# JiehongLin/SAM-6D

Measured on NVIDIA H100. Metric: poses/sec, higher is better.
Workload: dtype bf16

## Files before the change

### sam6d_b200/csrc/attn_tc.cu

```cuda
#include "epilogue.cuh"
#include "tc.cuh"

namespace {

constexpr int QT = 128, MAXK = 256;
constexpr int CONSUMERS = 256, NUM_THREADS = CONSUMERS + 128;
constexpr int REL_SLAB = 32 * 128;
constexpr int SCR_LD = 64;

struct AttnArgs {
  const float* bias;
  const void* rel_blob;
  const float* rel_unused;
  const void* q_rows;
  long long q_ld;
  int q_col0;
  const float* bv;
  void* out;
  long long out_ld;
  int H, Sq, Sk, N1;
  int Hs, Ws;
  int k_col0;
  float scale;
  int k_brows, k_row0, v_col0;
  float* lse;
  long long bias_ld;
};

template <int D>
__host__ __device__ constexpr int qkp_bytes(int N1) {
  return ((((D + 63) / 64) * (QT + N1) * 128 > 4 * QT * 128 ? ((D + 63) / 64) * (QT + N1) * 128 : 4 * QT * 128) + 1023) & ~1023;
}

template <int D, int BIAS_MODE, typename OT>
__global__ void __launch_bounds__(NUM_THREADS, 1) attn_tc_kernel(const __grid_constant__ CUtensorMap tmQ, const __grid_constant__ CUtensorMap tmK,
                                                const __grid_constant__ CUtensorMap tmVt, AttnArgs a) {
  constexpr int DS = (D + 63) / 64;
  constexpr int Q_SLAB = QT * 128, V_SLAB = D * 128, P_SLAB = QT * 128;
  const int K_SLAB = a.N1 * 128;
  extern __shared__ __align__(1024) uint8_t smem_raw[];
  uint8_t* smem = reinterpret_cast<uint8_t*>((reinterpret_cast<uintptr_t>(smem_raw) + 1023) & ~(uintptr_t)1023);
  uint8_t* q_s = smem;
  uint8_t* k_s = q_s + DS * Q_SLAB;
  uint8_t* p_s = smem;
  uint8_t* v_s = smem + qkp_bytes<D>(a.N1);
  uint8_t* rel_s = v_s + 4 * V_SLAB;
  float* scr = reinterpret_cast<float*>(rel_s + 2 * DS * REL_SLAB);
  __shared__ __align__(8) uint64_t load_bar;

  const int tid = threadIdx.x, warp = tid >> 5, lane = tid & 31;
  const int n0 = blockIdx.x * QT, h = blockIdx.y, b = blockIdx.z;
  const int nslab = (a.N1 + 63) / 64;

  if (tid == 0) {
    tc::mbar_init(&load_bar, 1);
    tc::mbar_fence_init();
  }
  s6_pdl_trigger();
  __syncthreads();
  s6_pdl_wait();

  if (warp >= CONSUMERS / 32) {
    tc::producer_regs();
    if (tid == CONSUMERS) {
      uint32_t bytes = (uint32_t)(DS * (QT * 128) + DS * (a.N1 * 128) + nslab * V_SLAB);
      if (BIAS_MODE == 2) bytes += 2 * DS * REL_SLAB;
      tc::mbar_arrive_expect_tx(&load_bar, bytes);
      if (BIAS_MODE == 2) tc::bulk_load_1d(rel_s, a.rel_blob, 2 * DS * REL_SLAB, &load_bar);
#pragma unroll
      for (int s = 0; s < DS; ++s) {
        tc::tma_load_2d(&tmQ, &load_bar, q_s + s * Q_SLAB, a.q_col0 + h * D + s * 64, b * a.Sq + n0);
        tc::tma_load_2d(&tmK, &load_bar, k_s + s * K_SLAB, a.k_col0 + h * D + s * 64, b * a.k_brows + a.k_row0);
      }
      for (int s = 0; s < nslab; ++s) tc::tma_load_2d(&tmVt, &load_bar, v_s + s * V_SLAB, a.v_col0 + s * 64, (b * a.H + h) * D);
    }
    return;
  }
  tc::consumer_regs();
  const int wg = warp >> 2, w = warp & 3;
  const int Sk = a.Sk;
  tc::mbar_wait(&load_bar, 0);
  float sacc[MAXK / 2];
  {
    const uint32_t q_addr = tc::smem_u32(q_s) + wg * (64 * 128), k_addr = tc::smem_u32(k_s);
    tc::wg_fence();
#pragma unroll
    for (int k = 0; k < D / 16; ++k) {
      const int sl = k >> 2, kk = k & 3;
      tc::wgmma_bf16<MAXK>(sacc, tc::wg_desc(q_addr + sl * Q_SLAB + kk * 32), tc::wg_desc(k_addr + sl * K_SLAB + kk * 32), k ? 1u : 0u);
    }
    tc::wg_commit();
    if (BIAS_MODE == 2) {
      float tacc[2][16];
#pragma unroll
      for (int t = 0; t < 2; ++t)
#pragma unroll
        for (int k = 0; k < D / 16; ++k) {
          const int sl = k >> 2, kk = k & 3;
          tc::wgmma_bf16<32>(tacc[t], tc::wg_desc(q_addr + sl * Q_SLAB + kk * 32),
                             tc::wg_desc(tc::smem_u32(rel_s + (t * DS + sl) * REL_SLAB) + kk * 32), k ? 1u : 0u);
        }
      tc::wg_commit();
      tc::wg_wait<0>();
#pragma unroll
      for (int t = 0; t < 2; ++t)
#pragma unroll
        for (int e = 0; e < 16; ++e) scr[(wg * 64 + tc::frag_row(e, w, lane)) * SCR_LD + t * 32 + tc::frag_col(e, lane)] = tacc[t][e];
      tc::named_bar(1 + wg, 128);
    } else {
      tc::wg_wait<0>();
    }
  }
  float mx[2] = {-INFINITY, -INFINITY};
#pragma unroll
  for (int hr = 0; hr < 2; ++hr) {
    const int r = wg * 64 + tc::frag_row(2 * hr, w, lane), n = n0 + r, nq = min(n, a.Sq - 1);
    const float* brow = nullptr;
    if (BIAS_MODE == 1) brow = a.bias + (((size_t)b * a.H + h) * a.Sq + nq) * Sk;
    if (BIAS_MODE == 4) brow = a.bias + (((size_t)b * a.H + h) * a.Sq + nq) * a.bias_ld;
    const float* trow = (BIAS_MODE == 2) ? scr + r * SCR_LD : nullptr;
    const int qh = (BIAS_MODE == 2) ? nq / a.Ws : 0, qw = (BIAS_MODE == 2) ? nq % a.Ws : 0;
#pragma unroll
    for (int j = 0; j < MAXK / 8; ++j) {
      const int col = tc::frag_col(4 * j, lane);
      float bb[2] = {0.f, 0.f};
      if (BIAS_MODE == 4 && col < Sk) { const float2 t = __ldg(reinterpret_cast<const float2*>(brow + col)); bb[0] = t.x; bb[1] = t.y; }
#pragma unroll
      for (int e = 0; e < 2; ++e) {
        const int c = col + e;
        float x = -INFINITY;
        if (c < Sk) {
          x = sacc[4 * j + 2 * hr + e];
          if (BIAS_MODE == 1) x += __ldg(brow + c);
          if (BIAS_MODE == 4) x += bb[e];
          x *= a.scale;
          if (BIAS_MODE == 2) { const int kh = c / a.Ws, kw = c - kh * a.Ws; x += trow[qh - kh + a.Hs - 1] + trow[32 + qw - kw + a.Ws - 1]; }
          mx[hr] = fmaxf(mx[hr], x);
        }
        sacc[4 * j + 2 * hr + e] = x;
      }
    }
    mx[hr] = tc::quad_max(mx[hr]);
  }
  tc::named_bar(3, CONSUMERS);
  float sum[2] = {0.f, 0.f};
#pragma unroll
  for (int j = 0; j < MAXK / 8; ++j) {
#pragma unroll
    for (int hr = 0; hr < 2; ++hr) {
      const int r = wg * 64 + tc::frag_row(2 * hr, w, lane), col = tc::frag_col(4 * j, lane);
      const float p0 = (col < Sk) ? __expf(sacc[4 * j + 2 * hr] - mx[hr]) : 0.f;
      const float p1 = (col + 1 < Sk) ? __expf(sacc[4 * j + 2 * hr + 1] - mx[hr]) : 0.f;
      sum[hr] += p0 + p1;
      *reinterpret_cast<uint32_t*>(p_s + (col >> 6) * P_SLAB + tc::sw128_offset(r, col & 63)) = tc::pack_bf16(p0, p1);
    }
  }
  tc::fence_proxy_async_smem();
  tc::named_bar(1 + wg, 128);
  float oacc[D / 2];
  {
    const uint32_t p_addr = tc::smem_u32(p_s) + wg * (64 * 128), v_addr = tc::smem_u32(v_s);
    tc::wg_fence();
    const int ksteps = a.N1 / 16;
    for (int k = 0; k < ksteps; ++k) {
      const int sl = k >> 2, kk = k & 3;
      tc::wgmma_bf16<D>(oacc, tc::wg_desc(p_addr + sl * P_SLAB + kk * 32), tc::wg_desc(v_addr + sl * V_SLAB + kk * 32), k ? 1u : 0u);
    }
    tc::wg_commit();
    tc::wg_wait<0>();
  }
  const int m_lim = b * a.Sq + a.Sq;
#pragma unroll
  for (int hr = 0; hr < 2; ++hr) {
    const float t = tc::quad_sum(sum[hr]), inv = 1.f / t;
    const int n = n0 + wg * 64 + tc::frag_row(2 * hr, w, lane), row = b * a.Sq + n;
    if (a.lse && n < a.Sq && (lane & 3) == 0) a.lse[((size_t)b * a.H + h) * a.Sq + n] = mx[hr] + __logf(t);
    if (row >= m_lim) continue;
    OT* orow = reinterpret_cast<OT*>(a.out) + (size_t)row * a.out_ld + h * D;
#pragma unroll
    for (int j = 0; j < D / 8; ++j) {
      const int col = tc::frag_col(4 * j, lane);
      float o0 = oacc[4 * j + 2 * hr] * inv, o1 = oacc[4 * j + 2 * hr + 1] * inv;
      if (a.bv) { o0 += __ldg(a.bv + h * D + col); o1 += __ldg(a.bv + h * D + col + 1); }
      epi::st2(orow + col, o0, o1);
    }
  }
}

template <int D, int BM, typename OT>
int launch(const CUtensorMap& tq, const CUtensorMap& tk, const CUtensorMap& tv, const AttnArgs& a, int B, cudaStream_t st) {
  constexpr int DS = (D + 63) / 64;
  size_t smem = (size_t)qkp_bytes<D>(a.N1) + (size_t)4 * D * 128 + 1024;
  if (BM == 2) smem += (size_t)2 * DS * REL_SLAB + (size_t)QT * SCR_LD * sizeof(float);
  if (smem > 227 * 1024) return S6_EINVAL;
  auto kern = attn_tc_kernel<D, BM, OT>;
  cudaError_t e = cudaFuncSetAttribute(kern, cudaFuncAttributeMaxDynamicSharedMemorySize, (int)smem);
  if (e != cudaSuccess) return (int)e;
  dim3 grid(s6_cdiv(a.Sq, QT), a.H, B);
  cudaError_t le = s6_launch_pdl(kern, grid, dim3(NUM_THREADS), smem, st, tq, tk, tv, a);
  if (le != cudaSuccess) return (int)le;
  return (int)cudaGetLastError();
}

__global__ void __launch_bounds__(256) transpose_tokens_kernel(const __nv_bfloat16* __restrict__ src, long long ld, int col0, int C,
                                                               int L, int N1, __nv_bfloat16* __restrict__ out) {
  __shared__ __nv_bfloat16 tile[64][66];
  const int w = blockIdx.z, c0 = blockIdx.y * 64, l0 = blockIdx.x * 64;
  const int tx = threadIdx.x & 63, ty = threadIdx.x >> 6;
  s6_pdl_trigger();
  s6_pdl_wait();
  for (int i = ty; i < 64; i += 4) {
    const int l = l0 + i, c = c0 + tx;
    tile[i][tx] = (l < L && c < C) ? src[((size_t)w * L + l) * ld + col0 + c] : __float2bfloat16(0.f);
  }
  __syncthreads();
  for (int i = ty; i < 64; i += 4) {
    const int c = c0 + i, l = l0 + tx;
    if (c < C && l < N1) out[((size_t)w * C + c) * N1 + l] = tile[tx][i];
  }
}

}

S6_API int sam6d_transpose_tokens_bf16(const void* src, long long ld, int col0, int C, int nB, int L, int N1, void* out, void* stream) {
  S6_REQUIRE(src && out && nB >= 0 && C > 0 && L > 0 && N1 >= L);
  if (nB == 0) return 0;
  S6_REQUIRE(nB <= 65535);
  dim3 grid(s6_cdiv(N1, 64), s6_cdiv(C, 64), nB);
  S6_CHECK(s6_launch_pdl(transpose_tokens_kernel, grid, dim3(256), 0, s6_stream(stream), reinterpret_cast<const __nv_bfloat16*>(src), ld,
                         col0, C, L, N1, reinterpret_cast<__nv_bfloat16*>(out)));
  S6_LAUNCH_CHECK();
  return 0;
}

namespace {
}

namespace {
int attn_tc_launch(const void* Q, long long q_ld, int q_col0, const void* K, long long k_ld, int k_col0, const void* Vt,
                   long long vt_ld, int B, int H, int Sq, int Sk, int head_dim, int bias_mode, const float* bias,
                   const void* rel_h, const float* rel_w, int Hs, int Ws, const float* bv, float scale, void* out,
                   int out_is_bf16, long long out_ld, int k_brows, int k_row0, int v_col0, float* lse, void* stream,
                   long long bias_ld = 0) {
  S6_REQUIRE(Q && K && Vt && out && B >= 0 && H > 0 && Sq > 0 && Sk > 0 && Sk <= MAXK);
  S6_REQUIRE((head_dim == 64 || head_dim == 80) && bias_mode >= 0 && bias_mode <= 4 && bias_mode != 3);
  if (bias_mode == 4)
    S6_REQUIRE(bias && head_dim == 64 && bias_ld >= Sk && (bias_ld % 4) == 0 && (reinterpret_cast<uintptr_t>(bias) & 15) == 0);
  S6_REQUIRE((q_ld % 8) == 0 && (k_ld % 8) == 0 && (vt_ld % 8) == 0 && (q_col0 % 8) == 0 && (k_col0 % 8) == 0);
  S6_REQUIRE(k_brows >= k_row0 + Sk && k_row0 >= 0 && v_col0 >= 0 && (v_col0 % 8) == 0);
  if (bias_mode == 1) S6_REQUIRE(bias != nullptr);
  if (bias_mode == 2) S6_REQUIRE(rel_h && Hs > 0 && Ws > 0 && Hs <= 16 && Ws <= 16 && Hs * Ws == Sk && Sq == Sk && (reinterpret_cast<uintptr_t>(rel_h) & 15) == 0);
  if (B == 0) return 0;
  S6_REQUIRE(B <= 65535 && H <= 65535);
  const int N1 = (Sk + 15) & ~15;
  S6_REQUIRE(vt_ld >= v_col0 + N1);
  CUtensorMap tq, tk, tv;
  int rc = tc::make_map_2d(&tq, Q, (long long)B * Sq, q_ld, q_ld, 64, QT);
  if (rc) return rc;
  rc = tc::make_map_2d(&tk, K, (long long)B * k_brows, k_ld, k_ld, 64, N1);
  if (rc) return rc;
  rc = tc::make_map_2d(&tv, Vt, (long long)B * H * head_dim, vt_ld, vt_ld, 64, head_dim);
  if (rc) return rc;
  AttnArgs a{bias, rel_h, rel_w, Q, q_ld, q_col0, bv, out, out_ld, H, Sq, Sk, N1, Hs, Ws, k_col0, scale, k_brows, k_row0, v_col0, lse, bias_ld};
  cudaStream_t st = s6_stream(stream);
#define ATT_LAUNCH(DD, MM) (out_is_bf16 ? launch<DD, MM, __nv_bfloat16>(tq, tk, tv, a, B, st) : launch<DD, MM, float>(tq, tk, tv, a, B, st))
  if (head_dim == 64) {
    if (bias_mode == 0) return ATT_LAUNCH(64, 0);
    if (bias_mode == 1) return ATT_LAUNCH(64, 1);
    if (bias_mode == 4) return ATT_LAUNCH(64, 4);
    return ATT_LAUNCH(64, 2);
  }
  if (bias_mode == 0) return ATT_LAUNCH(80, 0);
  if (bias_mode == 1) return ATT_LAUNCH(80, 1);
  return ATT_LAUNCH(80, 2);
#undef ATT_LAUNCH
}

__global__ void __launch_bounds__(256) attn_merge_key_kernel(const __nv_bfloat16* __restrict__ Q, long long q_ld, int q_col0,
                                                             const __nv_bfloat16* __restrict__ K, long long k_ld, int k_col0, int k_brows,
                                                             int key_row, const __nv_bfloat16* __restrict__ Vt, long long vt_ld, int key_col,
                                                             const float* __restrict__ lse, int B, int H, int Sq, float scale,
                                                             __nv_bfloat16* __restrict__ out, long long out_ld) {
  const long long w = (long long)blockIdx.x * 8 + (threadIdx.x >> 5);
  const int lane = threadIdx.x & 31;
  s6_pdl_trigger();
  s6_pdl_wait();
  if (w >= (long long)B * Sq * H) return;
  const int h = (int)(w % H);
  const long long bn = w / H;
  const int n = (int)(bn % Sq), b = (int)(bn / Sq);
  const __nv_bfloat162 q2 = *reinterpret_cast<const __nv_bfloat162*>(Q + (size_t)bn * q_ld + q_col0 + h * 64 + lane * 2);
  const __nv_bfloat162 k2 = *reinterpret_cast<const __nv_bfloat162*>(K + ((size_t)b * k_brows + key_row) * k_ld + k_col0 + h * 64 + lane * 2);
  float s = __bfloat162float(q2.x) * __bfloat162float(k2.x) + __bfloat162float(q2.y) * __bfloat162float(k2.y);
  s = warp_sum(s) * scale;
  const float l = lse[((size_t)b * H + h) * Sq + n];
  const float m = fmaxf(l, s), wp = __expf(l - m), wc = __expf(s - m), inv = 1.f / (wp + wc);
  const __nv_bfloat16* vrow = Vt + ((size_t)(b * H + h) * 64 + lane * 2) * vt_ld + key_col;
  const float v0 = __bfloat162float(vrow[0]), v1 = __bfloat162float(vrow[vt_ld]);
  __nv_bfloat162* o = reinterpret_cast<__nv_bfloat162*>(out + (size_t)bn * out_ld + h * 64 + lane * 2);
  const __nv_bfloat162 o2 = *o;
  *o = __floats2bfloat162_rn((wp * __bfloat162float(o2.x) + wc * v0) * inv, (wp * __bfloat162float(o2.y) + wc * v1) * inv);
}
}

S6_API int sam6d_attn_tc(const void* Q, long long q_ld, int q_col0, const void* K, long long k_ld, int k_col0, const void* Vt,
                         long long vt_ld, int B, int H, int Sq, int Sk, int head_dim, int bias_mode, const float* bias,
                         const void* rel_h, const float* rel_w, int Hs, int Ws, const float* bv, float scale, void* out,
                         int out_is_bf16, long long out_ld, void* stream) {
  return attn_tc_launch(Q, q_ld, q_col0, K, k_ld, k_col0, Vt, vt_ld, B, H, Sq, Sk, head_dim, bias_mode, bias, rel_h, rel_w, Hs, Ws, bv,
                        scale, out, out_is_bf16, out_ld, Sk, 0, 0, nullptr, stream);
}

S6_API int sam6d_attn_tc_bias_ld(const void* Q, long long q_ld, int q_col0, const void* K, long long k_ld, int k_col0, const void* Vt,
                                 long long vt_ld, int B, int H, int Sq, int Sk, int head_dim, const float* bias, long long bias_ld,
                                 float scale, void* out, int out_is_bf16, long long out_ld, void* stream) {
  return attn_tc_launch(Q, q_ld, q_col0, K, k_ld, k_col0, Vt, vt_ld, B, H, Sq, Sk, head_dim, 4, bias, nullptr, nullptr, 0, 0, nullptr,
                        scale, out, out_is_bf16, out_ld, Sk, 0, 0, nullptr, stream, bias_ld);
}

S6_API int sam6d_attn_tc_ex(const void* Q, long long q_ld, int q_col0, const void* K, long long k_ld, int k_col0, const void* Vt,
                            long long vt_ld, int B, int H, int Sq, int Sk, int head_dim, float scale, int k_brows, int k_row0, int v_col0,
                            float* lse, void* out, int out_is_bf16, long long out_ld, void* stream) {
  return attn_tc_launch(Q, q_ld, q_col0, K, k_ld, k_col0, Vt, vt_ld, B, H, Sq, Sk, head_dim, 0, nullptr, nullptr, nullptr, 0, 0, nullptr,
                        scale, out, out_is_bf16, out_ld, k_brows, k_row0, v_col0, lse, stream);
}

S6_API int sam6d_attn_merge_key(const void* Q, long long q_ld, int q_col0, const void* K, long long k_ld, int k_col0, int k_brows,
                                int key_row, const void* Vt, long long vt_ld, int key_col, const float* lse, int B, int H, int Sq,
                                float scale, void* out, long long out_ld, void* stream) {
  S6_REQUIRE(Q && K && Vt && lse && out && B >= 0 && H > 0 && Sq > 0 && (q_ld % 2) == 0 && (k_ld % 2) == 0 && (out_ld % 2) == 0 &&
             (q_col0 % 2) == 0 && (k_col0 % 2) == 0);
  if (B == 0) return 0;
  const long long warps = (long long)B * Sq * H;
  S6_CHECK(s6_launch_pdl(attn_merge_key_kernel, dim3(s6_cdiv(warps, 8)), dim3(256), 0, s6_stream(stream),
                         reinterpret_cast<const __nv_bfloat16*>(Q), q_ld, q_col0, reinterpret_cast<const __nv_bfloat16*>(K), k_ld, k_col0,
                         k_brows, key_row, reinterpret_cast<const __nv_bfloat16*>(Vt), vt_ld, key_col, lse, B, H, Sq, scale,
                         reinterpret_cast<__nv_bfloat16*>(out), out_ld));
  S6_LAUNCH_CHECK();
  return 0;
}
```

### sam6d_b200/csrc/geo_lut.cu

```cuda
#include <cuda_bf16.h>

#include "common.cuh"

namespace {

__device__ __forceinline__ uint32_t bf2_pack(float lo, float hi) {
  __nv_bfloat162 h = __floats2bfloat162_rn(lo, hi);
  return *reinterpret_cast<uint32_t*>(&h);
}

__device__ __forceinline__ void lut_pos(float x, float inv_h, int nent, int& row, float& t) {
  const float u = x * inv_h;
  int i = (int)u;
  i = max(0, min(i, nent - 2));
  t = u - (float)i;
  row = i * 32;
}
__device__ __forceinline__ void lut_lerp_f32(const uint4* __restrict__ tab, int row, float t, float v[8]) {
  const uint4 lo = tab[row], hi = tab[row + 32];
  const uint32_t l[4] = {lo.x, lo.y, lo.z, lo.w}, h[4] = {hi.x, hi.y, hi.z, hi.w};
#pragma unroll
  for (int k = 0; k < 4; ++k) {
    const float l0 = __uint_as_float(l[k] << 16), l1 = __uint_as_float(l[k] & 0xffff0000u);
    const float h0 = __uint_as_float(h[k] << 16), h1 = __uint_as_float(h[k] & 0xffff0000u);
    v[2 * k] = fmaf(t, h0 - l0, l0);
    v[2 * k + 1] = fmaf(t, h1 - l1, l1);
  }
}
__device__ __forceinline__ void unpack8(const uint4& a, float v[8]) {
  const uint32_t w[4] = {a.x, a.y, a.z, a.w};
#pragma unroll
  for (int k = 0; k < 4; ++k) { v[2 * k] = __uint_as_float(w[k] << 16); v[2 * k + 1] = __uint_as_float(w[k] & 0xffff0000u); }
}

__device__ __noinline__ uint4 slow_distance(float x, const float* __restrict__ div_term, const uint4* __restrict__ WdT,
                                            const float* __restrict__ bias, int lane) {
  float e[8];
#pragma unroll
  for (int q = 0; q < 4; ++q) sincosf(x * div_term[lane * 4 + q], &e[2 * q], &e[2 * q + 1]);
  float acc[8];
#pragma unroll
  for (int c = 0; c < 8; ++c) acc[c] = bias[lane * 8 + c];
  for (int s = 0; s < 32; ++s) {
#pragma unroll
    for (int q = 0; q < 8; ++q) {
      const float v = __shfl_sync(0xffffffffu, e[q], s);
      const uint4 w = WdT[(size_t)(s * 8 + q) * 32 + lane];
      const uint32_t ww[4] = {w.x, w.y, w.z, w.w};
#pragma unroll
      for (int i = 0; i < 4; ++i) {
        acc[2 * i] = fmaf(v, __uint_as_float(ww[i] << 16), acc[2 * i]);
        acc[2 * i + 1] = fmaf(v, __uint_as_float(ww[i] & 0xffff0000u), acc[2 * i + 1]);
      }
    }
  }
  return make_uint4(bf2_pack(acc[0], acc[1]), bf2_pack(acc[2], acc[3]), bf2_pack(acc[4], acc[5]), bf2_pack(acc[6], acc[7]));
}

constexpr int LUT_THREADS = 512, UNROLL = 2;
__global__ void __launch_bounds__(LUT_THREADS, 1) geo_embed_lut_kernel(const float4* __restrict__ T, long long npairs, int S,
                                                                      const uint4* __restrict__ tabA_g, int na, float inv_ha,
                                                                      const uint4* __restrict__ tabD_g, int nd, float inv_hd,
                                                                      const uint4* __restrict__ far, const float* __restrict__ div_term,
                                                                      const uint4* __restrict__ WdT, const float* __restrict__ bias,
                                                                      uint4* __restrict__ E) {
  extern __shared__ __align__(16) uint8_t smem_raw[];
  uint4* tabA = reinterpret_cast<uint4*>(smem_raw);
  uint4* tabD = tabA + na * 32;
  const int tid = threadIdx.x, lane = tid & 31, warp = tid >> 5;
  for (int u = tid; u < na * 32; u += LUT_THREADS) tabA[u] = tabA_g[u];
  for (int u = tid; u < nd * 32; u += LUT_THREADS) tabD[u] = tabD_g[u];
  __syncthreads();
  const float d_limit = (float)(nd - 1) / inv_hd;
  const long long nblocks = (npairs + 31) / 32;
  const long long SS = (long long)S * S;
  for (long long blk = (long long)blockIdx.x * (LUT_THREADS / 32) + warp; blk < nblocks; blk += (long long)gridDim.x * (LUT_THREADS / 32)) {
    const long long base = blk * 32;
    const int cnt = (int)min(32LL, npairs - base);
    float4 tv = make_float4(0.f, 0.f, 0.f, 0.f);
    if (lane < cnt) tv = T[base + lane];
    int r0, r1, r2, r3;
    float t0, t1, t2, t3;
    lut_pos(tv.x, inv_ha, na, r0, t0);
    lut_pos(tv.y, inv_ha, na, r1, t1);
    lut_pos(tv.z, inv_ha, na, r2, t2);
    lut_pos(tv.w, inv_hd, nd, r3, t3);
    if (!(tv.w < d_limit)) r3 = -1;
    const uint4* tabA_l = tabA + lane;
    const uint4* tabD_l = tabD + lane;
#pragma unroll UNROLL
    for (int j = 0; j < cnt; ++j) {
      const int q0 = __shfl_sync(0xffffffffu, r0, j), q1 = __shfl_sync(0xffffffffu, r1, j);
      const int q2 = __shfl_sync(0xffffffffu, r2, j), q3 = __shfl_sync(0xffffffffu, r3, j);
      const float w0 = __shfl_sync(0xffffffffu, t0, j), w1 = __shfl_sync(0xffffffffu, t1, j);
      const float w2 = __shfl_sync(0xffffffffu, t2, j), w3 = __shfl_sync(0xffffffffu, t3, j);
      uint4 dv;
      const bool in_table = q3 >= 0;
      if (!in_table) {
        const long long p = base + j;
        const long long c = p / SS;
        const int rem = (int)(p - c * SS), n = rem / S, m = rem - n * S;
        if (n == 0) dv = far[((c * 2 + 0) * S + m) * 32 + lane];
        else if (m == 0) dv = far[((c * 2 + 1) * S + n) * 32 + lane];
        else dv = slow_distance(__shfl_sync(0xffffffffu, tv.w, j), div_term, WdT, bias, lane);
      }
      float f0[8], f1[8], f2[8], fd[8];
      lut_lerp_f32(tabA_l, q0, w0, f0);
      lut_lerp_f32(tabA_l, q1, w1, f1);
      lut_lerp_f32(tabA_l, q2, w2, f2);
      if (in_table) lut_lerp_f32(tabD_l, q3, w3, fd);
      else unpack8(dv, fd);
#pragma unroll
      for (int k = 0; k < 8; ++k) fd[k] += fmaxf(fmaxf(f0[k], f1[k]), f2[k]);
      const uint4 o = make_uint4(bf2_pack(fd[0], fd[1]), bf2_pack(fd[2], fd[3]), bf2_pack(fd[4], fd[5]), bf2_pack(fd[6], fd[7]));
      E[(base + j) * 32 + lane] = o;
    }
  }
}

}

S6_API int sam6d_geo_embed_lut(const float* T, long long clouds, int S, const void* tabA, int na, float inv_ha, const void* tabD, int nd,
                               float inv_hd, const void* far, const float* div_term, const void* WdT_bf16, const float* bias, void* E,
                               void* stream) {
  S6_REQUIRE(T && tabA && tabD && far && div_term && WdT_bf16 && bias && E && clouds >= 0 && S > 0 && na >= 2 && nd >= 2);
  S6_REQUIRE(inv_ha > 0.f && inv_hd > 0.f && (long long)(na + nd) * 512 <= 200 * 1024);
  S6_REQUIRE(((reinterpret_cast<uintptr_t>(T) | reinterpret_cast<uintptr_t>(tabA) | reinterpret_cast<uintptr_t>(tabD) | reinterpret_cast<uintptr_t>(far) |
               reinterpret_cast<uintptr_t>(WdT_bf16) | reinterpret_cast<uintptr_t>(E)) & 15) == 0);
  const long long npairs = clouds * S * S;
  S6_REQUIRE(npairs < (1LL << 40));
  if (npairs == 0) return 0;
  const long long nblocks = (npairs + 31) / 32, want = (nblocks + LUT_THREADS / 32 - 1) / (LUT_THREADS / 32);
  int grid;
  S6_CHECK(s6_persistent_grid(want, 1, &grid));
  const int smem = (na + nd) * 512;
  S6_CHECK(cudaFuncSetAttribute(geo_embed_lut_kernel, cudaFuncAttributeMaxDynamicSharedMemorySize, smem));
  geo_embed_lut_kernel<<<grid, LUT_THREADS, smem, s6_stream(stream)>>>(
      reinterpret_cast<const float4*>(T), npairs, S, reinterpret_cast<const uint4*>(tabA), na, inv_ha, reinterpret_cast<const uint4*>(tabD),
      nd, inv_hd, reinterpret_cast<const uint4*>(far), div_term, reinterpret_cast<const uint4*>(WdT_bf16), bias, reinterpret_cast<uint4*>(E));
  S6_LAUNCH_CHECK();
  return 0;
}
```

Before: 2631.

## TMA-load bias tile into shared memory and split V load onto its own barrier

Result: faster. 2693, median of 6 (+2.4%).

```diff
diff --git a/sam6d_b200/csrc/attn_tc.cu b/sam6d_b200/csrc/attn_tc.cu
--- a/sam6d_b200/csrc/attn_tc.cu
+++ b/sam6d_b200/csrc/attn_tc.cu
@@ -25,6 +25,7 @@
   int k_brows, k_row0, v_col0;
   float* lse;
   long long bias_ld;
+  int bias_bc;
 };
 
 template <int D>
@@ -34,7 +35,7 @@
 
 template <int D, int BIAS_MODE, typename OT>
 __global__ void __launch_bounds__(NUM_THREADS, 1) attn_tc_kernel(const __grid_constant__ CUtensorMap tmQ, const __grid_constant__ CUtensorMap tmK,
-                                                const __grid_constant__ CUtensorMap tmVt, AttnArgs a) {
+                                                const __grid_constant__ CUtensorMap tmVt, const __grid_constant__ CUtensorMap tmB, AttnArgs a) {
   constexpr int DS = (D + 63) / 64;
   constexpr int Q_SLAB = QT * 128, V_SLAB = D * 128, P_SLAB = QT * 128;
   const int K_SLAB = a.N1 * 128;
@@ -46,7 +47,8 @@
   uint8_t* v_s = smem + qkp_bytes<D>(a.N1);
   uint8_t* rel_s = v_s + 4 * V_SLAB;
   float* scr = reinterpret_cast<float*>(rel_s + 2 * DS * REL_SLAB);
-  __shared__ __align__(8) uint64_t load_bar;
+  float* bias_s = reinterpret_cast<float*>(v_s + 4 * V_SLAB);
+  __shared__ __align__(8) uint64_t load_bar, bias_bar, v_bar;
 
   const int tid = threadIdx.x, warp = tid >> 5, lane = tid & 31;
   const int n0 = blockIdx.x * QT, h = blockIdx.y, b = blockIdx.z;
@@ -54,6 +56,8 @@
 
   if (tid == 0) {
     tc::mbar_init(&load_bar, 1);
+    tc::mbar_init(&v_bar, 1);
+    if (BIAS_MODE == 4) tc::mbar_init(&bias_bar, 1);
     tc::mbar_fence_init();
   }
   s6_pdl_trigger();
@@ -63,7 +67,7 @@
   if (warp >= CONSUMERS / 32) {
     tc::producer_regs();
     if (tid == CONSUMERS) {
-      uint32_t bytes = (uint32_t)(DS * (QT * 128) + DS * (a.N1 * 128) + nslab * V_SLAB);
+      uint32_t bytes = (uint32_t)(DS * (QT * 128) + DS * (a.N1 * 128));
       if (BIAS_MODE == 2) bytes += 2 * DS * REL_SLAB;
       tc::mbar_arrive_expect_tx(&load_bar, bytes);
       if (BIAS_MODE == 2) tc::bulk_load_1d(rel_s, a.rel_blob, 2 * DS * REL_SLAB, &load_bar);
@@ -72,7 +76,12 @@
         tc::tma_load_2d(&tmQ, &load_bar, q_s + s * Q_SLAB, a.q_col0 + h * D + s * 64, b * a.Sq + n0);
         tc::tma_load_2d(&tmK, &load_bar, k_s + s * K_SLAB, a.k_col0 + h * D + s * 64, b * a.k_brows + a.k_row0);
       }
-      for (int s = 0; s < nslab; ++s) tc::tma_load_2d(&tmVt, &load_bar, v_s + s * V_SLAB, a.v_col0 + s * 64, (b * a.H + h) * D);
+      if (BIAS_MODE == 4) {
+        tc::mbar_arrive_expect_tx(&bias_bar, (uint32_t)(QT * a.bias_bc * 4));
+        tc::tma_load_3d(&tmB, &bias_bar, bias_s, 0, n0, b * a.H + h);
+      }
+      tc::mbar_arrive_expect_tx(&v_bar, (uint32_t)(nslab * V_SLAB));
+      for (int s = 0; s < nslab; ++s) tc::tma_load_2d(&tmVt, &v_bar, v_s + s * V_SLAB, a.v_col0 + s * 64, (b * a.H + h) * D);
     }
     return;
   }
@@ -111,20 +120,21 @@
       tc::wg_wait<0>();
     }
   }
+  if (BIAS_MODE == 4) tc::mbar_wait(&bias_bar, 0);
   float mx[2] = {-INFINITY, -INFINITY};
 #pragma unroll
   for (int hr = 0; hr < 2; ++hr) {
     const int r = wg * 64 + tc::frag_row(2 * hr, w, lane), n = n0 + r, nq = min(n, a.Sq - 1);
     const float* brow = nullptr;
     if (BIAS_MODE == 1) brow = a.bias + (((size_t)b * a.H + h) * a.Sq + nq) * Sk;
-    if (BIAS_MODE == 4) brow = a.bias + (((size_t)b * a.H + h) * a.Sq + nq) * a.bias_ld;
+    if (BIAS_MODE == 4) brow = bias_s + r * a.bias_bc;
     const float* trow = (BIAS_MODE == 2) ? scr + r * SCR_LD : nullptr;
     const int qh = (BIAS_MODE == 2) ? nq / a.Ws : 0, qw = (BIAS_MODE == 2) ? nq % a.Ws : 0;
 #pragma unroll
     for (int j = 0; j < MAXK / 8; ++j) {
       const int col = tc::frag_col(4 * j, lane);
       float bb[2] = {0.f, 0.f};
-      if (BIAS_MODE == 4 && col < Sk) { const float2 t = __ldg(reinterpret_cast<const float2*>(brow + col)); bb[0] = t.x; bb[1] = t.y; }
+      if (BIAS_MODE == 4 && col < Sk) { const float2 t = *reinterpret_cast<const float2*>(brow + col); bb[0] = t.x; bb[1] = t.y; }
 #pragma unroll
       for (int e = 0; e < 2; ++e) {
         const int c = col + e;
@@ -160,6 +170,7 @@
   float oacc[D / 2];
   {
     const uint32_t p_addr = tc::smem_u32(p_s) + wg * (64 * 128), v_addr = tc::smem_u32(v_s);
+    tc::mbar_wait(&v_bar, 0);
     tc::wg_fence();
     const int ksteps = a.N1 / 16;
     for (int k = 0; k < ksteps; ++k) {
@@ -188,16 +199,17 @@
 }
 
 template <int D, int BM, typename OT>
-int launch(const CUtensorMap& tq, const CUtensorMap& tk, const CUtensorMap& tv, const AttnArgs& a, int B, cudaStream_t st) {
+int launch(const CUtensorMap& tq, const CUtensorMap& tk, const CUtensorMap& tv, const CUtensorMap& tb, const AttnArgs& a, int B, cudaStream_t st) {
   constexpr int DS = (D + 63) / 64;
   size_t smem = (size_t)qkp_bytes<D>(a.N1) + (size_t)4 * D * 128 + 1024;
   if (BM == 2) smem += (size_t)2 * DS * REL_SLAB + (size_t)QT * SCR_LD * sizeof(float);
+  if (BM == 4) smem += (size_t)QT * a.bias_bc * sizeof(float);
   if (smem > 227 * 1024) return S6_EINVAL;
   auto kern = attn_tc_kernel<D, BM, OT>;
   cudaError_t e = cudaFuncSetAttribute(kern, cudaFuncAttributeMaxDynamicSharedMemorySize, (int)smem);
   if (e != cudaSuccess) return (int)e;
   dim3 grid(s6_cdiv(a.Sq, QT), a.H, B);
-  cudaError_t le = s6_launch_pdl(kern, grid, dim3(NUM_THREADS), smem, st, tq, tk, tv, a);
+  cudaError_t le = s6_launch_pdl(kern, grid, dim3(NUM_THREADS), smem, st, tq, tk, tv, tb, a);
   if (le != cudaSuccess) return (int)le;
   return (int)cudaGetLastError();
 }
@@ -234,6 +246,17 @@
 }
 
 namespace {
+int make_bias_map(CUtensorMap* map, const float* ptr, long long planes, int Sq, long long ld, int box_cols) {
+  tc::EncodeFn enc = tc::get_encode();
+  if (!enc) return 999;
+  cuuint64_t gdim[3] = {(cuuint64_t)ld, (cuuint64_t)Sq, (cuuint64_t)planes};
+  cuuint64_t gstride[2] = {(cuuint64_t)ld * sizeof(float), (cuuint64_t)Sq * ld * sizeof(float)};
+  cuuint32_t box[3] = {(cuuint32_t)box_cols, (cuuint32_t)QT, 1};
+  cuuint32_t estr[3] = {1, 1, 1};
+  CUresult r = enc(map, CU_TENSOR_MAP_DATA_TYPE_FLOAT32, 3, const_cast<float*>(ptr), gdim, gstride, box, estr, CU_TENSOR_MAP_INTERLEAVE_NONE,
+                   CU_TENSOR_MAP_SWIZZLE_NONE, CU_TENSOR_MAP_L2_PROMOTION_L2_256B, CU_TENSOR_MAP_FLOAT_OOB_FILL_NONE);
+  return r == CUDA_SUCCESS ? 0 : 1000 + (int)r;
+}
 }
 
 namespace {
@@ -261,9 +284,15 @@
   if (rc) return rc;
   rc = tc::make_map_2d(&tv, Vt, (long long)B * H * head_dim, vt_ld, vt_ld, 64, head_dim);
   if (rc) return rc;
-  AttnArgs a{bias, rel_h, rel_w, Q, q_ld, q_col0, bv, out, out_ld, H, Sq, Sk, N1, Hs, Ws, k_col0, scale, k_brows, k_row0, v_col0, lse, bias_ld};
+  AttnArgs a{bias, rel_h, rel_w, Q, q_ld, q_col0, bv, out, out_ld, H, Sq, Sk, N1, Hs, Ws, k_col0, scale, k_brows, k_row0, v_col0, lse, bias_ld,
+             (Sk + 3) & ~3};
+  CUtensorMap tb = tq;
+  if (bias_mode == 4) {
+    rc = make_bias_map(&tb, bias, (long long)B * H, Sq, bias_ld, a.bias_bc);
+    if (rc) return rc;
+  }
   cudaStream_t st = s6_stream(stream);
-#define ATT_LAUNCH(DD, MM) (out_is_bf16 ? launch<DD, MM, __nv_bfloat16>(tq, tk, tv, a, B, st) : launch<DD, MM, float>(tq, tk, tv, a, B, st))
+#define ATT_LAUNCH(DD, MM) (out_is_bf16 ? launch<DD, MM, __nv_bfloat16>(tq, tk, tv, tb, a, B, st) : launch<DD, MM, float>(tq, tk, tv, tb, a, B, st))
   if (head_dim == 64) {
     if (bias_mode == 0) return ATT_LAUNCH(64, 0);
     if (bias_mode == 1) return ATT_LAUNCH(64, 1);
diff --git a/sam6d_b200/csrc/geo_lut.cu b/sam6d_b200/csrc/geo_lut.cu
--- a/sam6d_b200/csrc/geo_lut.cu
+++ b/sam6d_b200/csrc/geo_lut.cu
@@ -57,7 +57,7 @@
   return make_uint4(bf2_pack(acc[0], acc[1]), bf2_pack(acc[2], acc[3]), bf2_pack(acc[4], acc[5]), bf2_pack(acc[6], acc[7]));
 }
 
-constexpr int LUT_THREADS = 512, UNROLL = 2;
+constexpr int LUT_THREADS = 768, UNROLL = 2;
 __global__ void __launch_bounds__(LUT_THREADS, 1) geo_embed_lut_kernel(const float4* __restrict__ T, long long npairs, int S,
                                                                       const uint4* __restrict__ tabA_g, int na, float inv_ha,
                                                                       const uint4* __restrict__ tabD_g, int nd, float inv_hd,
```
